# pytorch/ELF

Hardware: AMD Instinct MI355X
Metric: mcts_rollouts_per_sec (self-play, 19x19 Go, 8192 rollouts/move, bs 16) (higher is better)
Workload: dtype f32; 1 GPU; BASELINE configs[2]: MCTS self-play bs=16, 8192 rollouts/move, 20x256 fp16 net on PyTorch-ROCm, 2048 games/GPU in 1 group(s), window crosses a move boundary; games_per_gpu=2048, groups=1, board_size=19, mcts_threads=1, net_dtype=fp16, moves_in_window=2048, nodes_per_game=12288, node_bytes=6626, live_nodes=6241478, largest_tree=8184

## Files before the change

elf_amd/_lib.py:

```python
import ctypes as C
import os

HERE = os.path.dirname(os.path.abspath(__file__))
LIB_PATH = os.path.join(HERE, "lib", "libelf_amd.so")
ZOBRIST_BIN = os.path.join(HERE, "data", "zobrist21.bin")

_lib = None

KERNEL_SOURCES = ("go_board.cuh", "mcts.cuh", "train.cuh", "stl_emul.h", "engine_host.h", "elf_amd.hip", "mcts_capi.hip", "train_capi.hip",
                  "net_epilogue.hip", "Makefile")


def kernel_source_hash():
    import hashlib
    h = hashlib.sha256()
    for name in KERNEL_SOURCES:
        with open(os.path.join(HERE, "csrc", name), "rb") as f:
            h.update(name.encode() + b"\0" + f.read() + b"\0")
    return h.hexdigest()[:16]

_vp, _i, _i64, _f, _sz = C.c_void_p, C.c_int, C.c_int64, C.c_float, C.c_size_t
SIGNATURES = {
    "elfgo_create": (_i, [_i, _i, _i, _vp, C.POINTER(_vp)]),
    "elfgo_destroy": (_i, [_vp]),
    "elfgo_board_size": (_i, [_vp]),
    "elfgo_capacity": (_i, [_vp]),
    "elfgo_slot_bytes": (_sz, [_vp]),
    "elfgo_sync": (_i, [_vp, _vp]),
    "elfgo_reset": (_i, [_vp, _vp, _i, _vp]),
    "elfgo_copy": (_i, [_vp, _vp, _vp, _i, _vp]),
    "elfgo_forward": (_i, [_vp, _vp, _vp, _i, _vp, _vp]),
    "elfgo_legal_mask": (_i, [_vp, _vp, _i, _vp, _vp]),
    "elfgo_extract_agz": (_i, [_vp, _vp, _vp, _i, _vp, _i64, _vp]),
    "elfgo_extract_agz_fmt": (_i, [_vp, _vp, _vp, _i, _vp, _i64, _i, _vp]),
    "elfgo_evaluate": (_i, [_vp, _vp, _i, _f, _vp, _vp]),
    "elfgo_info": (_i, [_vp, _vp, _i, _vp, _vp]),
    "elfgo_export_board": (_i, [_vp, _vp, _i, _vp, _vp, _vp]),
    "elfgo_playout": (_i, [_vp, _vp, _vp, _i, _i, _vp, _vp]),
    "elfgo_setup": (_i, [_vp, _vp, _vp, _vp, _i, _vp, _vp]),
    "elfgo_area_map": (_i, [_vp, _vp, _i, _vp, _vp]),
    "elfgo_ladder_map": (_i, [_vp, _vp, _i, _vp, _vp, _vp]),
    "elfgo_own_create": (_i, [_vp, _i, C.POINTER(_vp)]),
    "elfgo_own_destroy": (_i, [_vp]),
    "elfgo_own_scratch_bytes": (_sz, [_vp]),
    "elfgo_own_run": (_i, [_vp, _vp, _vp, _i, _i, _i, _f, _vp, _vp, _vp]),
    "elfmcts_create": (_i, [_vp, _i, _i, _i, _vp, C.POINTER(_vp)]),
    "elfmcts_destroy": (_i, [_vp]),
    "elfmcts_set_options": (_i, [_vp, _vp]),
    "elfmcts_set_feature_format": (_i, [_vp, _i]),
    "elfmcts_get_feature_format": (_i, [_vp, C.POINTER(_i)]),
    "elfmcts_max_rollouts_per_step": (_i, []),
    "elfmcts_set_game_mask": (_i, [_vp, _vp]),
    "elfmcts_set_required_versions": (_i, [_vp, _vp]),
    "elfmcts_num_games": (_i, [_vp]),
    "elfmcts_edge_stride": (_i, [_vp]),
    "elfmcts_node_bytes": (_sz, [_vp]),
    "elfmcts_tree_bytes_per_game": (_sz, [_i, _i]),
    "elfmcts_tree_bytes_per_game2": (_sz, [_i, _i, _i, _i, _i]),
    "elfmcts_pool_info": (_i, [_vp, _vp, _i]),
    "elfmcts_count_live": (_i, [_vp, _vp]),
    "elfmcts_num_threads": (_i, [_vp]),
    "elfmcts_thread_draws": (_i, [_vp, _vp, _vp]),
    "elfmcts_clear": (_i, [_vp, _vp, _i, _vp]),
    "elfmcts_set_root": (_i, [_vp, _vp, _vp]),
    "elfmcts_set_d4": (_i, [_vp, _vp, _vp]),
    "elfmcts_dirichlet": (_i, [_vp, _vp, _vp, _f, _vp]),
    "elfmcts_select": (_i, [_vp, _vp, _vp, _i64, _vp, _vp]),
    "elfmcts_expand": (_i, [_vp, _vp, _i64, _vp, _vp, _i, _vp]),
    "elfmcts_root": (_i, [_vp, _vp, _vp, _vp, _vp, _vp, _vp, _vp]),
    "elfmcts_advance": (_i, [_vp, _vp, _vp]),
    "elfmcts_validate": (_i, [_vp, _vp]),
    "elfmcts_node_visits": (_i, [_vp, _vp]),
    "elfsp_create": (_i, [_vp, _i, _vp, C.POINTER(_vp)]),
    "elfsp_destroy": (_i, [_vp]),
    "elfsp_engine": (_vp, [_vp]),
    "elfsp_mcts": (_vp, [_vp]),
    "elfsp_ts_requests_deferred": (_i64, [_vp]),
    "elfsp_ts_games_deferred": (_i, [_vp]),
    "elfsp_max_rows": (_i, [_vp]),
    "elfsp_max_rows_actor": (_i, [_vp, _i]),
    "elfsp_mcts_actor": (_vp, [_vp, _i]),
    "elfsp_begin_step2": (_i, [_vp, _vp, _i64, _vp, _vp]),
    "elfsp_end_step2": (_i, [_vp, _vp, _i64, _vp, _vp, _vp]),
    "elfsp_last_rows2": (_i, [_vp, _vp]),
    "elfsp_set_request2": (_i, [_vp, _vp]),
    "elfsp_set_request3": (_i, [_vp, _vp, _vp]),
    "elfrec_sgf_parse": (_i, [_i, C.c_char_p, _vp, _vp, _i, _vp]),
    "elfrec_sgf_setup": (_i, [_i, C.c_char_p, _vp, _vp]),
    "elfrec_game_sgf": (_i64, [_vp, _vp, _i, _vp, _i, _f, C.c_char_p, C.c_char_p, C.c_char_p, C.c_char_p, _sz]),
    "elfrec_record_to_sgf": (_i64, [_vp, C.c_char_p, C.c_char_p, C.c_char_p, _sz, C.c_char_p, _sz]),
    "elfrec_client_create": (_i, [C.c_char_p, C.POINTER(_vp)]),
    "elfrec_client_destroy": (_i, [_vp]),
    "elfrec_client_feed": (_i, [_vp, C.c_char_p]),
    "elfrec_client_update_state": (_i, [_vp, _vp]),
    "elfrec_client_size": (_i, [_vp]),
    "elfrec_client_dump_and_clear": (_i64, [_vp, C.c_char_p, _sz]),
    "elfrec_parse_request_seq": (_i, [C.c_char_p, _vp, C.POINTER(_i64), _vp]),
    "elfrec_request_seq_to_json": (_i64, [_vp, _vp, _i64, C.c_char_p, _sz]),
    "elfsp_thread_states": (_i, [_vp, _vp, _i]),
    "elfrq_create": (_i, [_i, _i, _i, C.c_uint32, C.POINTER(_vp)]),
    "elfrq_destroy": (_i, [_vp]),
    "elfrq_insert": (_i, [_vp, C.c_int32, C.c_int32, _i, C.POINTER(C.c_int32)]),
    "elfrq_sizes": (_i, [_vp, _vp]),
    "elfrq_set_threads": (_i, [_vp, _i, _i64, C.c_uint64]),
    "elfrq_draw": (_i, [_vp, _i, _i, _vp, _vp, _vp]),
    "elfsp_progress": (_i, [_vp, _vp]),
    "elfsp_set_pick_seed": (_i, [_vp, C.c_uint32]),
    "elfsp_game_actor": (_i, [_vp, _i]),
    "elfsp_begin_step": (_i, [_vp, _vp, _i64, C.POINTER(_i), _vp]),
    "elfsp_end_step": (_i, [_vp, _vp, _i64, _vp, _vp, _vp]),
    "elfsp_last_rows": (_i, [_vp, C.POINTER(_i)]),
    "elfsp_set_request": (_i, [_vp, _i64, _i64, _f, _f, _i]),
    "elfsp_take_game_starts": (_i, [_vp, C.POINTER(_i64), C.POINTER(_i64)]),
    "elfsp_stats": (_i, [_vp, _vp]),
    "elfsp_games_finished": (_i64, [_vp]),
    "elfsp_search_log": (_i, [_vp, _i, _i, _vp, _vp, _vp, _vp, _vp]),
    "elfsp_play": (_i, [_vp, _vp, _vp]),
    "elfsp_preload": (_i, [_vp, _vp, _i, _i, _vp]),
    "elfsp_restart": (_i, [_vp, _vp, _i, _vp]),
    "elfsp_setup": (_i, [_vp, _vp, _i, _vp, _vp, _vp]),
    "elfsp_undo": (_i, [_vp, _vp, _i, _i, _vp]),
    "elfsp_finish": (_i, [_vp, _vp, _i, _i, _vp]),
    "elfsp_take_finished": (_i, [_vp, _vp, _i]),
    "elfsp_last_score": (_i, [_vp, _vp]),
    "elfsp_last_moves": (_i, [_vp, _vp]),
    "elfsp_records_pending": (_i, [_vp]),
    "elfsp_pop_record": (_i, [_vp, _vp, _sz, C.POINTER(_sz)]),
    "elftrain_create": (_i, [_vp, _i, _i, _i, C.c_uint32, C.POINTER(_vp)]),
    "elftrain_destroy": (_i, [_vp]),
    "elftrain_capacity": (_i, [_vp]),
    "elftrain_max_moves": (_i, [_vp]),
    "elftrain_num_records": (_i, [_vp]),
    "elftrain_put": (_i, [_vp, _i, _vp, _i, _f, _i64, _vp, _i, _vp, _i]),
    "elftrain_put_async": (_i, [_vp, _i, _vp, _i, _f, _i64, _vp, _i, _vp, _i, _vp]),
    "elftrain_set_keep_states": (_i, [_vp, _i]),
    "elftrain_draw": (_i, [_vp, _i, _i, _vp, _vp, _vp, _vp]),
    "elftrain_extract": (_i, [_vp, _vp, _vp, _vp, _i, _vp, _vp]),
    "elfrec_coords_to_sgfstr": (_i, [_i, _vp, _i, _vp, _sz]),
    "elfrec_sgfstr_to_coords": (_i, [_i, C.c_char_p, _vp, _i]),
    "elfrec_record_to_json": (_i, [_vp, _vp, _i, _vp, _i, _vp, _i, _f, _i, _i, C.c_uint64, C.c_uint64, _vp, _sz]),
    "elfrec_record_to_json2": (_i, [_vp, _vp, _vp, _i, _vp, _i, _vp, _i, _f, _i, _i, C.c_uint64, C.c_uint64, _vp, _sz]),
    "elfrec_quantise_policy": (_i, [_i, _vp, _vp, _i, _vp]),
    "elfnet_bias_act_f16": (_i, [_vp, _vp, _vp, _i64, _i, _i, _vp]),
    "elfnet_bias_act_bf16": (_i, [_vp, _vp, _vp, _i64, _i, _i, _vp]),
    "elfnet_conv3x3_f16": (_i, [_vp, _vp, _vp, _vp, _vp, _i64, _i, _i, _i, _i, _i, _i, _vp]),
    "elfnet_conv3x3_in_f16": (_i, [_vp, _vp, _vp, _vp, _i64, _i, _i, _i, _i, _i, _vp]),
    "elfnet_heads_workspace": (_sz, [_i64, _i, _i]),
    "elfnet_heads_f16": (_i, [_vp, _vp, _i64, _i, _i, _vp, _i64, _vp, _vp, _vp, _sz, _vp]),
    "elfgo_set_device": (_i, [_i]),
    "elfgo_get_device": (_i, [C.POINTER(_i)]),
    "elfgo_mem_info": (_i, [_i, C.POINTER(_sz), C.POINTER(_sz)]),
    "elfgo_pointer_kind": (_i, [_vp, C.POINTER(_i)]),
    "elfgo_memcpy2d_async": (_i, [_vp, _sz, _vp, _sz, _sz, _sz, _vp]),
    "elfgo_stream_sync": (_i, [_vp]),
    "elfgo_malloc": (_i, [C.POINTER(_vp), _sz]),
    "elfgo_free": (_i, [_vp]),
    "elfgo_memcpy_h2d": (_i, [_vp, _vp, _sz]),
    "elfgo_memcpy_d2h": (_i, [_vp, _vp, _sz]),
    "elfgo_error_string": (C.c_char_p, [_i]),
    "elfgo_version": (C.c_char_p, []),
}


class ElfNetHeads(C.Structure):
    _fields_ = [(n, _vp) for n in ("pconv_w", "pconv_b", "vconv_w", "vconv_b", "pi_w", "pi_b", "v1_w", "v1_b", "v2_w", "v2_b")] + \
               [("channels", C.c_int32), ("value_hidden", C.c_int32)]


def lib():
    global _lib
    if _lib is None:
        if not os.path.exists(LIB_PATH):
            raise ImportError(
                "elf_amd: %s not built. Run `python -c 'import __graft_entry__ as g; g.build()'` "
                "(or make -C elf_amd/csrc). There is no CPU fallback." % LIB_PATH
            )
        L = C.CDLL(LIB_PATH)
        for name, (res, args) in SIGNATURES.items():
            f = getattr(L, name)
            f.restype = res
            f.argtypes = args
        _lib = L
    return _lib


class ElfGoError(RuntimeError):
    pass


def check(status):
    if status != 0:
        raise ElfGoError("libelf_amd status %d: %s" % (status, lib().elfgo_error_string(status).decode()))
```

elf_amd/csrc/net_conv.hip:

```cpp
#include <hip/hip_runtime.h>
#include <stdint.h>

#include <array>

#if !__has_include("ck/ck.hpp")
#error "net_conv.hip needs Composable Kernel's headers (ck/ck.hpp, shipped with ROCm under <rocm>/include/ck): there is no build of libelf_amd.so without the fused trunk convolution"
#endif
#include "ck/ck.hpp"
#include "ck/tensor_operation/gpu/device/convolution_forward_specialization.hpp"
#include "ck/tensor_operation/gpu/device/gemm_specialization.hpp"
#include "ck/tensor_operation/gpu/device/impl/device_grouped_conv_fwd_multiple_abd_xdl_cshuffle.hpp"
#include "ck/tensor_operation/gpu/device/tensor_layout.hpp"
#include "ck/tensor_operation/gpu/element/element_wise_operation.hpp"

#include "../../include/elf_amd.h"

namespace {

using F16 = ck::half_t;
using F32 = float;
template <ck::index_t... Is>
using S = ck::Sequence<Is...>;
using PassThrough = ck::tensor_operation::element_wise::PassThrough;
namespace lay = ck::tensor_layout::convolution;

struct BiasResAct {
  int relu;
  template <typename E, typename C, typename D0>
  __host__ __device__ void operator()(E& e, const C& c, const D0& bias) const {
    float v = ck::type_convert<float>(ck::type_convert<F16>(c));
    v += ck::type_convert<float>(bias);
    if (relu) v = fmaxf(v, 0.0f);
    e = ck::type_convert<E>(v);
  }
  template <typename E, typename C, typename D0, typename D1>
  __host__ __device__ void operator()(E& e, const C& c, const D0& bias, const D1& res) const {
    float v = ck::type_convert<float>(ck::type_convert<F16>(c));
    v += ck::type_convert<float>(bias);
    v += ck::type_convert<float>(res);
    if (relu) v = fmaxf(v, 0.0f);
    e = ck::type_convert<E>(v);
  }
};

constexpr auto kConvDefault = ck::tensor_operation::device::ConvolutionForwardSpecialization::Default;
constexpr auto kMNKPadding = ck::tensor_operation::device::GemmSpecialization::MNKPadding;

template <typename DsLayout, typename DsTypes>
using ConvA = ck::tensor_operation::device::DeviceGroupedConvFwdMultipleABD_Xdl_CShuffle<
    2, lay::NHWGC, lay::GKYXC, DsLayout, lay::NHWGK, F16, F16, F32, F16, DsTypes, F16, PassThrough, PassThrough, BiasResAct,
    kConvDefault, kMNKPadding, 1, 256, 256, 128, 32, 8, 8, 32, 32, 4, 2,
    S<4, 64, 1>, S<1, 0, 2>, S<1, 0, 2>, 2, 8, 8, 1,
    S<4, 64, 1>, S<1, 0, 2>, S<1, 0, 2>, 2, 8, 8, 1,
    1, 1, S<1, 32, 1, 8>, 8>;

using DsBias = ck::Tuple<lay::G_K>;
using DsBiasRes = ck::Tuple<lay::G_K, lay::NHWGK>;
using T1 = ck::Tuple<F16>;
using T2 = ck::Tuple<F16, F16>;

struct DevGuard {
  int prev = -1;
  explicit DevGuard(int dev) {
    int cur = -1;
    if (hipGetDevice(&cur) == hipSuccess && cur != dev && hipSetDevice(dev) == hipSuccess) prev = cur;
  }
  ~DevGuard() { if (prev >= 0) (void)hipSetDevice(prev); }
  DevGuard(const DevGuard&) = delete;
  DevGuard& operator=(const DevGuard&) = delete;
};

struct Shape { int n, h, w, c, k; };

template <typename Op, int ND>
int run(const void* x, const void* w, const std::array<const void*, ND>& ds, void* y, const Shape& s, int relu, hipStream_t stream,
        bool launch) {
  using A5 = std::array<ck::index_t, 5>;
  using A2 = std::array<ck::index_t, 2>;
  const int n = s.n, h = s.h, wd = s.w, c = s.c, k = s.k;
  const A5 xl{1, n, c, h, wd}, xs{c, h * wd * c, 1, wd * c, c};
  const A5 wl{1, k, c, 3, 3}, ws{k * 9 * c, 9 * c, 1, 3 * c, c};
  const A5 yl{1, n, k, h, wd}, ys{k, h * wd * k, 1, wd * k, k};
  const A5 bs{k, 0, 1, 0, 0};
  std::array<A5, ND> dl, dst;
  dl[0] = yl; dst[0] = bs;
  if (ND == 2) { dl[ND - 1] = yl; dst[ND - 1] = ys; }
  const A2 one{1, 1};
  try {
    auto arg = Op::MakeArgument(x, w, ds, y, xl, xs, wl, ws, dl, dst, yl, ys, one, one, one, one, PassThrough{}, PassThrough{},
                                BiasResAct{relu});
    if (!Op::IsSupportedArgument(arg)) return ELFGO_E_BADARG;
    if (!launch) return 0;
    auto inv = Op::MakeInvoker();
    (void)inv.Run(arg, StreamConfig{stream, false});
  } catch (...) {
    hipError_t e = hipGetLastError();
    return e == hipSuccess ? (int)hipErrorLaunchFailure : (int)e;
  }
  hipError_t e = hipGetLastError();
  return e == hipSuccess ? 0 : (int)e;
}

}

extern "C" __attribute__((visibility("hidden"))) int elfnet_conv3x3_native_f16(const void* x, const void* w, const void* bias,
                                                                               const void* res, void* y, int64_t rows, int h, int wd,
                                                                               int c, int k, int relu, hipStream_t stream);

extern "C" int elfnet_conv3x3_f16(const void* x, const void* w, const void* bias, const void* res, void* y, int64_t rows, int h, int wd,
                                  int c, int k, int relu, int algo, void* stream) {
  if (!x || !w || !bias || !y || rows < 0 || h <= 0 || wd <= 0 || c <= 0 || k <= 0) return ELFGO_E_BADARG;
  if ((c & 7) != 0 || (k & 7) != 0 || (algo != 0 && algo != 1)) return ELFGO_E_BADARG;
  if ((((uintptr_t)x | (uintptr_t)w | (uintptr_t)bias | (uintptr_t)res | (uintptr_t)y) & 15) != 0) return ELFGO_E_BADARG;
  if (y == x || y == res) return ELFGO_E_BADARG;
  const int64_t cmax = c > k ? c : k;
  if (rows * h * wd * cmax >= ((int64_t)1 << 30) || (int64_t)k * 9 * c >= ((int64_t)1 << 30)) return ELFGO_E_BADARG;
  if (rows == 0) return 0;
  hipPointerAttribute_t at;
  if (hipPointerGetAttributes(&at, x) != hipSuccess) { (void)hipGetLastError(); return ELFGO_E_BADARG; }
  DevGuard _dg(at.device);
  const Shape s{(int)rows, h, wd, c, k};
  hipStream_t st = (hipStream_t)stream;
  if (algo == 1) return elfnet_conv3x3_native_f16(x, w, bias, res, y, rows, h, wd, c, k, relu, st);
  if (res) return run<ConvA<DsBiasRes, T2>, 2>(x, w, {bias, res}, y, s, relu, st, true);
  return run<ConvA<DsBias, T1>, 1>(x, w, {bias}, y, s, relu, st, true);
}
```

elf_amd/csrc/net_conv3x3.hip:

```cpp
#include <hip/hip_runtime.h>
#include <stdint.h>

#include "../../include/elf_amd.h"


namespace {

typedef _Float16 half8 __attribute__((ext_vector_type(8)));
typedef _Float16 half4 __attribute__((ext_vector_type(4)));
typedef float floatx16 __attribute__((ext_vector_type(16)));

constexpr int kTileM = 256;
constexpr int kTileN = 256;
constexpr int kThreads = 512;
constexpr int kOperandBytes = 256 * 128;
constexpr int kBufBytes = 2 * kOperandBytes;
constexpr int kLdsBytes = 2 * kBufBytes;

__device__ __attribute__((aligned(128))) unsigned char g_zero_line[128] = {0};

typedef const __attribute__((address_space(1))) void* gptr_t;
typedef __attribute__((address_space(3))) void* lptr_t;

__device__ __forceinline__ void stage16(const char* src, char* lds_base) {
  __builtin_amdgcn_global_load_lds((gptr_t)src, (lptr_t)lds_base, 16, 0, 0);
}

template <int kN, bool kLgkm>
__device__ __forceinline__ void wait_staged() {
  if constexpr (kLgkm) asm volatile("s_waitcnt vmcnt(%0) lgkmcnt(0)" ::"n"(kN) : "memory");
  else asm volatile("s_waitcnt vmcnt(%0)" ::"n"(kN) : "memory");
}
__device__ __forceinline__ void raw_barrier() {
  __builtin_amdgcn_s_barrier();
  asm volatile("" ::: "memory");
  __builtin_amdgcn_sched_barrier(0);
}
template <int kV> struct Mode { static constexpr int v = kV; };

template <bool kHasRes>
__global__ __launch_bounds__(kThreads, 2) void k_conv3x3_f16(const char* __restrict__ x, const char* __restrict__ w,
                                                             const _Float16* __restrict__ bias, const _Float16* __restrict__ res,
                                                             _Float16* __restrict__ y, int M, int H, int W, int Cin, int K, int relu) {
  __shared__ __attribute__((aligned(128))) char lds[kLdsBytes];
  const int tid = threadIdx.x, lane = tid & 63, wv = __builtin_amdgcn_readfirstlane(tid >> 6);
  const int kbase = blockIdx.y * kTileN;
  const int tile = blockIdx.x;

  uint32_t xoff[4], woff[4], xmask[4];
  const unsigned char* zsrc = g_zero_line + (lane & 7) * 16;
#pragma unroll
  for (int j = 0; j < 4; ++j) {
    const int hf = j >> 1, i = j & 1;
    const int r = i * 128 + hf * 64 + wv * 8 + (lane >> 3);
    const int p = tile * kTileM + r;
    uint32_t m = 0;
    if (p < M) {
      const int rem = p % (H * W), hh = rem / W, ww = rem - hh * W;
#pragma unroll
      for (int tap = 0; tap < 9; ++tap) {
        const int dy = tap / 3 - 1, dx = tap % 3 - 1;
        if ((unsigned)(hh + dy) < (unsigned)H && (unsigned)(ww + dx) < (unsigned)W) m |= 1u << tap;
      }
    }
    xmask[j] = m;
    xoff[j] = (uint32_t)p * (uint32_t)(Cin * 2) + (((lane & 7) ^ ((r >> 1) & 7)) << 4);
    const int rw = (i * 2 + (wv >> 2)) * 64 + hf * 32 + (wv & 3) * 8 + (lane >> 3);
    woff[j] = (uint32_t)(kbase + rw) * (uint32_t)(9 * Cin * 2) + (((lane & 7) ^ ((rw >> 1) & 7)) << 4);
  }
  auto stage_x = [&](int hf, int tap, int kc, int buf) {
    const int dy = tap / 3 - 1, dx = tap - (tap / 3) * 3 - 1;
    const uint32_t d = (uint32_t)((dy * W + dx) * Cin * 2 + kc * 128);
#pragma unroll
    for (int i = 0; i < 2; ++i)
      stage16(((xmask[hf * 2 + i] >> tap) & 1) ? x + (uint32_t)(xoff[hf * 2 + i] + d) : (const char*)zsrc,
              lds + buf * kBufBytes + (i * 128 + hf * 64 + wv * 8) * 128);
  };
  auto stage_w = [&](int hf, int tap, int kc, int buf) {
    const uint32_t d = (uint32_t)(tap * Cin * 2 + kc * 128);
#pragma unroll
    for (int i = 0; i < 2; ++i)
      stage16(w + (uint32_t)(woff[hf * 2 + i] + d),
              lds + buf * kBufBytes + kOperandBytes + ((i * 2 + (wv >> 2)) * 64 + hf * 32 + (wv & 3) * 8) * 128);
  };

  const int wm = wv >> 2, wn = wv & 3;
  const int fr = lane & 31, fh = lane >> 5;
  const int sw = (fr >> 1) & 7;
  const int xrow = (wm * 128 + fr) * 128;
  const int wrow = kOperandBytes + (wn * 64 + fr) * 128;
  int cs[4];
#pragma unroll
  for (int kk = 0; kk < 4; ++kk) cs[kk] = (((kk >> 1) * 4 + fh * 2 + (kk & 1)) ^ sw) << 4;
  auto ldx = [&](const char* b, int mt, int kk) { return *(const half8*)(b + xrow + mt * 4096 + cs[kk]); };
  auto ldw = [&](const char* b, int nt, int kk) { return *(const half8*)(b + wrow + nt * 4096 + cs[kk]); };

  floatx16 acc[4][2];
#pragma unroll
  for (int mt = 0; mt < 4; ++mt)
#pragma unroll
    for (int nt = 0; nt < 2; ++nt)
#pragma unroll
      for (int e = 0; e < 16; ++e) acc[mt][nt][e] = 0.0f;

  const int kchunks = Cin >> 6, ktiles = 9 * kchunks;
  half8 xf[2][4], wa[4], wb[4];
  int tap1 = 0, kc1 = 1, tap2 = 0, kc2 = 2;
  if (kchunks == 1) { tap1 = 1; kc1 = 0; tap2 = 2; kc2 = 0; }
  else if (kchunks == 2) { tap2 = 1; kc2 = 0; }
  stage_x(0, 0, 0, 0); stage_w(0, 0, 0, 0); stage_w(1, 0, 0, 0); stage_x(1, 0, 0, 0);
  stage_x(0, tap1, kc1, 1); stage_w(0, tap1, kc1, 1); stage_w(1, tap1, kc1, 1);
  wait_staged<8, false>();
  raw_barrier();

  auto ktile = [&](auto mode, int t) {
    constexpr int kMode = decltype(mode)::v;
    const int cur = t & 1, nxt = cur ^ 1;
    const char* b = lds + cur * kBufBytes;
#pragma unroll
    for (int kk = 0; kk < 4; ++kk) {
      wa[kk] = ldw(b, 0, kk);
      xf[0][kk] = ldx(b, 0, kk);
      xf[1][kk] = ldx(b, 1, kk);
      wb[kk] = ldw(b, 1, kk);
    }
    if constexpr (kMode <= 1) stage_x(1, tap1, kc1, nxt);
    wait_staged<kMode == 2 ? 0 : 8, true>();
    raw_barrier();
    __builtin_amdgcn_s_setprio(1);
#pragma unroll
    for (int kk = 0; kk < 4; ++kk) {
      acc[0][0] = __builtin_amdgcn_mfma_f32_32x32x16_f16(wa[kk], xf[0][kk], acc[0][0], 0, 0, 0);
      acc[1][0] = __builtin_amdgcn_mfma_f32_32x32x16_f16(wa[kk], xf[1][kk], acc[1][0], 0, 0, 0);
      acc[0][1] = __builtin_amdgcn_mfma_f32_32x32x16_f16(wb[kk], xf[0][kk], acc[0][1], 0, 0, 0);
      acc[1][1] = __builtin_amdgcn_mfma_f32_32x32x16_f16(wb[kk], xf[1][kk], acc[1][1], 0, 0, 0);
    }
    __builtin_amdgcn_s_setprio(0);
    __builtin_amdgcn_sched_barrier(0);
    raw_barrier();
#pragma unroll
    for (int kk = 0; kk < 4; ++kk) {
      xf[0][kk] = ldx(b, 2, kk);
      xf[1][kk] = ldx(b, 3, kk);
    }
    if constexpr (kMode == 0) { stage_x(0, tap2, kc2, cur); stage_w(0, tap2, kc2, cur); stage_w(1, tap2, kc2, cur); }
    wait_staged<kMode == 0 ? 8 : kMode == 1 ? 2 : 0, true>();
    raw_barrier();
    __builtin_amdgcn_s_setprio(1);
#pragma unroll
    for (int kk = 0; kk < 4; ++kk) {
      acc[2][0] = __builtin_amdgcn_mfma_f32_32x32x16_f16(wa[kk], xf[0][kk], acc[2][0], 0, 0, 0);
      acc[3][0] = __builtin_amdgcn_mfma_f32_32x32x16_f16(wa[kk], xf[1][kk], acc[3][0], 0, 0, 0);
      acc[2][1] = __builtin_amdgcn_mfma_f32_32x32x16_f16(wb[kk], xf[0][kk], acc[2][1], 0, 0, 0);
      acc[3][1] = __builtin_amdgcn_mfma_f32_32x32x16_f16(wb[kk], xf[1][kk], acc[3][1], 0, 0, 0);
    }
    __builtin_amdgcn_s_setprio(0);
    __builtin_amdgcn_sched_barrier(0);
    raw_barrier();
  };
  const int late = __builtin_amdgcn_readfirstlane(tid >> 8);
  if (late) raw_barrier();
  for (int t = 0; t < ktiles - 2; ++t) {
    ktile(Mode<0>{}, t);
    tap1 = tap2; kc1 = kc2;
    if (++kc2 == kchunks) { kc2 = 0; ++tap2; }
  }
  ktile(Mode<1>{}, ktiles - 2);
  ktile(Mode<2>{}, ktiles - 1);
  if (!late) raw_barrier();

  __syncthreads();
#pragma unroll
  for (int mt = 0; mt < 4; ++mt)
#pragma unroll
    for (int nt = 0; nt < 2; ++nt) {
      const int pos = wm * 128 + mt * 32 + fr;
#pragma unroll
      for (int g = 0; g < 4; ++g) {
        const int ch = wn * 64 + nt * 32 + g * 8 + fh * 4;
        half4 hv;
#pragma unroll
        for (int e = 0; e < 4; ++e) hv[e] = (_Float16)acc[mt][nt][g * 4 + e];
        *(half4*)(lds + pos * 512 + (((ch >> 3) ^ (pos & 31)) << 4) + ((ch >> 2) & 1) * 8) = hv;
      }
    }
  const int q = tid & 31;
  const half8 bv = *(const half8*)(bias + kbase + q * 8);
  if constexpr (kHasRes) {
    half8 rv[16];
#pragma unroll
    for (int it = 0; it < 16; ++it) {
      const int p = tile * kTileM + it * 16 + (tid >> 5);
      rv[it] = *(const half8*)(res + (size_t)(p < M ? p : M - 1) * K + kbase + q * 8);
    }
    __syncthreads();
#pragma unroll
    for (int it = 0; it < 16; ++it) {
      const int pos = it * 16 + (tid >> 5);
      const int p = tile * kTileM + pos;
      const half8 cv = *(const half8*)(lds + pos * 512 + ((q ^ (pos & 31)) << 4));
      half8 ov;
#pragma unroll
      for (int e = 0; e < 8; ++e) {
        float v = (float)cv[e];
        v += (float)bv[e];
        v += (float)rv[it][e];
        if (relu) v = fmaxf(v, 0.0f);
        ov[e] = (_Float16)v;
      }
      if (p < M) *(half8*)(y + (size_t)p * K + kbase + q * 8) = ov;
    }
  } else {
    __syncthreads();
#pragma unroll 4
    for (int it = 0; it < 16; ++it) {
      const int pos = it * 16 + (tid >> 5);
      const int p = tile * kTileM + pos;
      if (p < M) {
        const half8 cv = *(const half8*)(lds + pos * 512 + ((q ^ (pos & 31)) << 4));
        half8 ov;
#pragma unroll
        for (int e = 0; e < 8; ++e) {
          float v = (float)cv[e];
          v += (float)bv[e];
          if (relu) v = fmaxf(v, 0.0f);
          ov[e] = (_Float16)v;
        }
        *(half8*)(y + (size_t)p * K + kbase + q * 8) = ov;
      }
    }
  }
}

}

extern "C" __attribute__((visibility("hidden"))) int elfnet_conv3x3_native_f16(const void* x, const void* w, const void* bias,
                                                                               const void* res, void* y, int64_t rows, int h, int wd,
                                                                               int c, int k, int relu, hipStream_t stream) {
  if ((c & 63) != 0 || (k & 255) != 0) return ELFGO_E_BADARG;
  const int64_t m = rows * h * wd;
  const dim3 grid((unsigned)((m + kTileM - 1) / kTileM), (unsigned)(k / kTileN));
  if (res)
    hipLaunchKernelGGL(k_conv3x3_f16<true>, grid, dim3(kThreads), 0, stream, (const char*)x, (const char*)w, (const _Float16*)bias,
                       (const _Float16*)res, (_Float16*)y, (int)m, h, wd, c, k, relu);
  else
    hipLaunchKernelGGL(k_conv3x3_f16<false>, grid, dim3(kThreads), 0, stream, (const char*)x, (const char*)w, (const _Float16*)bias,
                       (const _Float16*)nullptr, (_Float16*)y, (int)m, h, wd, c, k, relu);
  hipError_t e = hipGetLastError();
  return e == hipSuccess ? 0 : (int)e;
}
```

include/elf_amd.h:

```cpp
#ifndef ELF_AMD_H_
#define ELF_AMD_H_
#include <stddef.h>
#include <stdint.h>

#ifdef __cplusplus
extern "C" {
#endif

typedef struct ElfGoEngine ElfGoEngine;

#define ELFGO_E_BADARG (-1)
#define ELFGO_E_BADSIZE (-2)
#define ELFGO_E_NOMEM (-3)
#define ELFGO_E_NODATA (-4)

#define ELFGO_INFO_WORDS 16

int elfgo_create(int board_size, int capacity, int device, const uint64_t* zobrist_host, ElfGoEngine** out);
int elfgo_destroy(ElfGoEngine* e);
int elfgo_board_size(const ElfGoEngine* e);
int elfgo_capacity(const ElfGoEngine* e);
size_t elfgo_slot_bytes(const ElfGoEngine* e);
int elfgo_sync(ElfGoEngine* e, void* stream);

// ... 115 lines not shown
  int32_t following_pass;
  int32_t reserved1;
} ElfSpOptions;
#define ELFSP_PICK_MOST_VISITED 0
#define ELFSP_PICK_STRONGEST_PRIOR 1
#define ELFSP_PICK_UNIFORM_RANDOM 2
#define ELFSP_ACTOR_BLACK 0
#define ELFSP_ACTOR_WHITE 1

typedef struct ElfSpSearch {
  int32_t game, move_played, best_action, total_visits, n_edges;
  float root_value, max_score, predicted_value;
} ElfSpSearch;

int elfsp_create(const ElfSpOptions* opt, int device, const uint64_t* zobrist_host, ElfSelfPlay** out);
int elfsp_destroy(ElfSelfPlay* sp);
ElfGoEngine* elfsp_engine(ElfSelfPlay* sp);
ElfMcts* elfsp_mcts(ElfSelfPlay* sp);
int64_t elfsp_ts_requests_deferred(const ElfSelfPlay* sp);
int elfsp_ts_games_deferred(const ElfSelfPlay* sp);
int elfsp_max_rows(const ElfSelfPlay* sp);
int elfsp_max_rows_actor(const ElfSelfPlay* sp, int actor);
ElfMcts* elfsp_mcts_actor(ElfSelfPlay* sp, int actor);
int elfsp_begin_step(ElfSelfPlay* sp, void* s_dst, int64_t stride_elems, int* n_rows, void* stream);
int elfsp_end_step(ElfSelfPlay* sp, const float* pi, int64_t pi_stride_floats, const float* value, const int64_t* rv, void* stream);
int elfsp_last_rows(ElfSelfPlay* sp, int* n_rows);
int elfsp_begin_step2(ElfSelfPlay* sp, void* const* s_dst, int64_t stride_elems, int* n_rows, void* stream);
int elfsp_end_step2(ElfSelfPlay* sp, const float* const* pi, int64_t pi_stride_floats, const float* const* value,
                    const int64_t* const* rv, void* stream);
int elfsp_last_rows2(ElfSelfPlay* sp, int* n_rows);
typedef struct ElfTsOptions {
  int32_t max_num_moves, num_threads, num_rollouts_per_thread, num_rollouts_per_batch;
  int32_t verbose, verbose_time, persistent_tree, pick_method ;
  int64_t seed;
  float root_epsilon, root_alpha;
  int32_t virtual_loss;
  int32_t use_prior, unexplored_q_zero, root_unexplored_q_zero;
  float c_puct;
  char log_prefix[60];
} ElfTsOptions;
typedef struct ElfSpRequest {
  int64_t black_ver, white_ver;
  float black_resign_thres, white_resign_thres, never_resign_prob;
  int32_t num_game_thread_used;
  int32_t player_swap;
  int32_t async;
  int32_t client_type;
} ElfSpRequest;
int elfsp_set_request2(ElfSelfPlay* sp, const ElfSpRequest* request);
int elfsp_set_request3(ElfSelfPlay* sp, const ElfSpRequest* request, const ElfTsOptions* mcts_opt);
int elfsp_set_request(ElfSelfPlay* sp, int64_t black_ver, int64_t white_ver, float resign_thres, float never_resign_prob, int async);
int elfsp_set_pick_seed(ElfSelfPlay* sp, uint32_t seed);
int elfsp_progress(const ElfSelfPlay* sp, int64_t* out6);
int elfsp_game_actor(const ElfSelfPlay* sp, int game);
int elfsp_take_game_starts(ElfSelfPlay* sp, int64_t* black_ver, int64_t* white_ver);
int elfsp_stats(ElfSelfPlay* sp, int64_t* out);
int elfsp_play(ElfSelfPlay* sp, const int32_t* moves_host, void* stream);
int elfsp_preload(ElfSelfPlay* sp, const uint16_t* moves_host, int n, int move_to, void* stream);
int elfsp_setup(ElfSelfPlay* sp, const int32_t* games_host, int n, const uint8_t* stones_host,
                const uint8_t* next_player_host, void* stream);
int elfsp_undo(ElfSelfPlay* sp, const int32_t* games_host, int n, int count, void* stream);
#define ELFSP_FR_RESIGN 0
#define ELFSP_FR_TWO_PASSES 1
#define ELFSP_FR_MAX_STEP 2
#define ELFSP_FR_CLEAR 3
#define ELFSP_FR_ILLEGAL 4
int elfsp_finish(ElfSelfPlay* sp, const int32_t* games_host, int n, int reason, void* stream);
int elfsp_restart(ElfSelfPlay* sp, const int32_t* games_host, int n, void* stream);
int elfsp_take_finished(ElfSelfPlay* sp, float* out_host, int cap);
int elfsp_last_score(const ElfSelfPlay* sp, float* out_host);
int elfsp_last_moves(const ElfSelfPlay* sp, int32_t* out_host);
int elfsp_records_pending(const ElfSelfPlay* sp);
int elfsp_pop_record(ElfSelfPlay* sp, char* buf, size_t cap, size_t* len);
int64_t elfsp_games_finished(const ElfSelfPlay* sp);
int elfsp_search_log(const ElfSelfPlay* sp, int first, int n, ElfSpSearch* rec, int32_t* coord, int32_t* visits, float* prior,
                     float* reward);

typedef struct ElfReplay ElfReplay;

typedef struct ElfTrainBatch {
  void* s;
  int64_t s_stride;
  int32_t s_format;
  int32_t num_future_actions;
  int64_t* offline_a;
  float* winner;
  float* mcts_scores;
  float* predicted_value;
  int32_t* move_idx;
  int32_t* num_move;
  int32_t* aug_code;
  int64_t* selfplay_ver;
} ElfTrainBatch;

int elftrain_create(ElfGoEngine* e, int capacity, int max_moves, int with_policies, uint32_t seed, ElfReplay** out);
int elftrain_destroy(ElfReplay* r);
int elftrain_capacity(const ElfReplay* r);
int elftrain_max_moves(const ElfReplay* r);
int elftrain_num_records(const ElfReplay* r);
int elftrain_put(ElfReplay* r, int slot, const uint16_t* moves_host, int num_moves, float reward, int64_t black_ver,
                 const uint8_t* policies_host, int num_policies, const float* values_host, int num_values);
int elftrain_put_async(ElfReplay* r, int slot, const uint16_t* moves_host, int num_moves, float reward, int64_t black_ver,
                       const uint8_t* policies_host, int num_policies, const float* values_host, int num_values, void* stream);
int elftrain_set_keep_states(ElfReplay* r, int on);
int elftrain_draw(ElfReplay* r, int n, int num_future_actions, int32_t* rec, int32_t* move_to, int32_t* d4, void* stream);
typedef struct ElfSgfHeader {
  int32_t size, handi, winner ;
  float komi, win_margin;
} ElfSgfHeader;
int elfrec_sgf_parse(int board_size, const char* text, int32_t* players, uint16_t* coords, int cap, ElfSgfHeader* header);
int elfrec_sgf_setup(int board_size, const char* text, uint8_t* stones, ElfSgfHeader* header);
int64_t elfrec_game_sgf(const ElfSpOptions* opt, const uint16_t* moves, int num_moves, const float* values, int num_values,
                        float final_value, const char* filename, const char* git_hash, const char* git_staged, char* out, size_t cap);
int64_t elfrec_record_to_sgf(const ElfSpOptions* opt, const char* record_json, const char* prefix, char* name_out, size_t name_cap,
                             char* out, size_t cap);
typedef struct ElfThreadState {
  int32_t thread_id, seq, move_idx, reserved;
  int64_t black, white;
} ElfThreadState;
typedef struct ElfClientRecords ElfClientRecords;
int elfrec_client_create(const char* identity, ElfClientRecords** out);
int elfrec_client_destroy(ElfClientRecords* c);
int elfrec_client_feed(ElfClientRecords* c, const char* record_json);
int elfrec_client_update_state(ElfClientRecords* c, const ElfThreadState* state);
int elfrec_client_size(const ElfClientRecords* c);
int64_t elfrec_client_dump_and_clear(ElfClientRecords* c, char* out, size_t cap);
int elfrec_parse_request_seq(const char* json_text, ElfSpRequest* request, int64_t* seq, ElfTsOptions* mcts_opt);
int64_t elfrec_request_seq_to_json(const ElfSpRequest* request, const ElfTsOptions* mcts_opt, int64_t seq, char* out, size_t cap);
int elfsp_thread_states(const ElfSelfPlay* sp, ElfThreadState* out, int capacity);
typedef struct ElfReaderQueues ElfReaderQueues;
int elfrq_create(int num_reader, int queue_min_size, int queue_max_size, uint32_t insert_seed, ElfReaderQueues** out);
int elfrq_destroy(ElfReaderQueues* q);
int elfrq_insert(ElfReaderQueues* q, int32_t slot, int32_t num_moves, int black_win, int32_t* evicted);
int elfrq_sizes(const ElfReaderQueues* q, int32_t* per_queue);
int elfrq_set_threads(ElfReaderQueues* q, int num_threads, int64_t seed, uint64_t job_hash);
int elfrq_draw(ElfReaderQueues* q, int num_acts, int num_future_actions, int32_t* slot, int32_t* move_to, int32_t* d4);
int elftrain_extract(ElfReplay* r, const int32_t* rec, const int32_t* move_to, const int32_t* d4, int n, const ElfTrainBatch* out,
                     void* stream);

int elfrec_coords_to_sgfstr(int board_size, const uint16_t* coords, int n, char* out, size_t cap);
int elfrec_sgfstr_to_coords(int board_size, const char* sgf, uint16_t* out, int cap);
int elfrec_record_to_json(const ElfSpOptions* opt, const uint16_t* moves, int num_moves, const uint8_t* policies, int num_policies,
                          const float* values, int num_values, float reward, int never_resign, int seq, uint64_t thread_id,
                          uint64_t timestamp, char* out, size_t cap);
int elfrec_record_to_json2(const ElfSpOptions* opt, const ElfSpRequest* request, const uint16_t* moves, int num_moves,
                           const uint8_t* policies, int num_policies, const float* values, int num_values, float reward, int never_resign,
                           int seq, uint64_t thread_id, uint64_t timestamp, char* out, size_t cap);
int elfrec_quantise_policy(int board_size, const int32_t* coord, const float* prob, int n, uint8_t* out);

int elfnet_bias_act_f16(void* x, const void* bias, const void* res, int64_t rows, int channels, int relu, void* stream);
int elfnet_bias_act_bf16(void* x, const void* bias, const void* res, int64_t rows, int channels, int relu, void* stream);
int elfnet_conv3x3_f16(const void* x, const void* w, const void* bias, const void* res, void* y,
                       int64_t rows, int h, int wd, int c, int k, int relu, int algo, void* stream);

int elfnet_conv3x3_in_f16(const void* x, const void* w, const void* bias, void* y,
                          int64_t rows, int h, int wd, int c, int k, int relu, void* stream);

typedef struct ElfNetHeads {
  const void *pconv_w, *pconv_b;
  const void *vconv_w, *vconv_b;
  const void *pi_w, *pi_b;
  const void *v1_w, *v1_b;
  const void *v2_w, *v2_b;
  int32_t channels, value_hidden;
} ElfNetHeads;
size_t elfnet_heads_workspace(int64_t rows, int h, int wd);
int elfnet_heads_f16(const void* act, const ElfNetHeads* hd, int64_t rows, int h, int wd,
                     float* pi, int64_t pi_stride, float* value, float* logits,
                     void* workspace, size_t workspace_bytes, void* stream);

int elfgo_set_device(int device);
int elfgo_get_device(int* device);
int elfgo_mem_info(int device, size_t* free_bytes, size_t* total_bytes);
int elfgo_pointer_kind(const void* p, int* device);
int elfgo_memcpy2d_async(void* dst, size_t dst_pitch, const void* src, size_t src_pitch, size_t width_bytes, size_t rows, void* stream);
int elfgo_stream_sync(void* stream);
int elfgo_malloc(void** dptr, size_t bytes);
int elfgo_free(void* dptr);
int elfgo_memcpy_h2d(void* dst, const void* src_host, size_t bytes);
int elfgo_memcpy_d2h(void* dst_host, const void* src, size_t bytes);
const char* elfgo_error_string(int status);
const char* elfgo_version(void);

#ifdef __cplusplus
}
#endif
#endif
```

Measured before the change: 61010 rollouts/s.

## Split tail-wave conv3x3 tiles into half-width work items to balance last round

The native conv3x3 kernel now maps a flat work-item index to (tile, column, half). When the final wave across the device's CUs would be at most half full, the remaining tiles are split into two half-N-width items computed by a kNT=1 variant of the tile routine. This targets the wave-quantization tail in the trunk convolution at bs16 MCTS shapes. In exchange it adds more templated kernel code, a plan query API and a device CU-count lookup, and half tiles reload the full activation operand.

New measurement: 62050 rollouts/s, median of 6. +1.7%, better.

```diff
diff --git a/elf_amd/_lib.py b/elf_amd/_lib.py
--- a/elf_amd/_lib.py
+++ b/elf_amd/_lib.py
@@ -144,6 +144,8 @@
     "elfnet_bias_act_f16": (_i, [_vp, _vp, _vp, _i64, _i, _i, _vp]),
     "elfnet_bias_act_bf16": (_i, [_vp, _vp, _vp, _i64, _i, _i, _vp]),
     "elfnet_conv3x3_f16": (_i, [_vp, _vp, _vp, _vp, _vp, _i64, _i, _i, _i, _i, _i, _i, _vp]),
+    "elfnet_conv3x3_f16_width": (_i, [_vp, _vp, _vp, _vp, _vp, _i64, _i, _i, _i, _i, _i, _i, _i, _vp]),
+    "elfnet_conv3x3_f16_plan": (_i64, [_i64, _i, _i, _i64, C.POINTER(_i), C.POINTER(_i), C.POINTER(_i)]),
     "elfnet_conv3x3_in_f16": (_i, [_vp, _vp, _vp, _vp, _i64, _i, _i, _i, _i, _i, _vp]),
     "elfnet_heads_workspace": (_sz, [_i64, _i, _i]),
     "elfnet_heads_f16": (_i, [_vp, _vp, _i64, _i, _i, _vp, _i64, _vp, _vp, _vp, _sz, _vp]),
diff --git a/elf_amd/csrc/net_conv.hip b/elf_amd/csrc/net_conv.hip
--- a/elf_amd/csrc/net_conv.hip
+++ b/elf_amd/csrc/net_conv.hip
@@ -105,12 +105,18 @@
 
 extern "C" __attribute__((visibility("hidden"))) int elfnet_conv3x3_native_f16(const void* x, const void* w, const void* bias,
                                                                                const void* res, void* y, int64_t rows, int h, int wd,
-                                                                               int c, int k, int relu, hipStream_t stream);
+                                                                               int c, int k, int relu, int round_width,
+                                                                               hipStream_t stream);
 
 extern "C" int elfnet_conv3x3_f16(const void* x, const void* w, const void* bias, const void* res, void* y, int64_t rows, int h, int wd,
                                   int c, int k, int relu, int algo, void* stream) {
+  return elfnet_conv3x3_f16_width(x, w, bias, res, y, rows, h, wd, c, k, relu, algo, 0, stream);
+}
+
+extern "C" int elfnet_conv3x3_f16_width(const void* x, const void* w, const void* bias, const void* res, void* y, int64_t rows, int h,
+                                        int wd, int c, int k, int relu, int algo, int round_width, void* stream) {
   if (!x || !w || !bias || !y || rows < 0 || h <= 0 || wd <= 0 || c <= 0 || k <= 0) return ELFGO_E_BADARG;
-  if ((c & 7) != 0 || (k & 7) != 0 || (algo != 0 && algo != 1)) return ELFGO_E_BADARG;
+  if ((c & 7) != 0 || (k & 7) != 0 || (algo != 0 && algo != 1) || round_width < 0) return ELFGO_E_BADARG;
   if ((((uintptr_t)x | (uintptr_t)w | (uintptr_t)bias | (uintptr_t)res | (uintptr_t)y) & 15) != 0) return ELFGO_E_BADARG;
   if (y == x || y == res) return ELFGO_E_BADARG;
   const int64_t cmax = c > k ? c : k;
@@ -121,7 +127,7 @@
   DevGuard _dg(at.device);
   const Shape s{(int)rows, h, wd, c, k};
   hipStream_t st = (hipStream_t)stream;
-  if (algo == 1) return elfnet_conv3x3_native_f16(x, w, bias, res, y, rows, h, wd, c, k, relu, st);
+  if (algo == 1) return elfnet_conv3x3_native_f16(x, w, bias, res, y, rows, h, wd, c, k, relu, round_width, st);
   if (res) return run<ConvA<DsBiasRes, T2>, 2>(x, w, {bias, res}, y, s, relu, st, true);
   return run<ConvA<DsBias, T1>, 1>(x, w, {bias}, y, s, relu, st, true);
 }
diff --git a/elf_amd/csrc/net_conv3x3.hip b/elf_amd/csrc/net_conv3x3.hip
--- a/elf_amd/csrc/net_conv3x3.hip
+++ b/elf_amd/csrc/net_conv3x3.hip
@@ -1,5 +1,7 @@
 #include <hip/hip_runtime.h>
 #include <stdint.h>
+
+#include <atomic>
 
 #include "../../include/elf_amd.h"
 
@@ -38,14 +40,28 @@
 }
 template <int kV> struct Mode { static constexpr int v = kV; };
 
-template <bool kHasRes>
-__global__ __launch_bounds__(kThreads, 2) void k_conv3x3_f16(const char* __restrict__ x, const char* __restrict__ w,
-                                                             const _Float16* __restrict__ bias, const _Float16* __restrict__ res,
-                                                             _Float16* __restrict__ y, int M, int H, int W, int Cin, int K, int relu) {
-  __shared__ __attribute__((aligned(128))) char lds[kLdsBytes];
+struct WorkItem { int tile, col, half; };
+__host__ __device__ inline WorkItem work_item(int id, int tiles, int nfull) {
+  int half = -1;
+  if (id >= nfull) {
+    const int e = id - nfull;
+    id = nfull + (e >> 1);
+    half = e & 1;
+  }
+  const int col = id / tiles;
+  return WorkItem{id - col * tiles, col, half};
+}
+__host__ __device__ inline int full_items(int64_t total, int64_t width) {
+  const int64_t r = total % width;
+  return (int)(total >= width && r > 0 && 2 * r <= width ? total - r : total);
+}
+
+template <bool kHasRes, int kNT>
+__device__ __forceinline__ void conv_tile(char* lds, const char* __restrict__ x, const char* __restrict__ w,
+                                          const _Float16* __restrict__ bias, const _Float16* __restrict__ res,
+                                          _Float16* __restrict__ y, int M, int H, int W, int Cin, int K, int relu, int tile,
+                                          int kbase) {
   const int tid = threadIdx.x, lane = tid & 63, wv = __builtin_amdgcn_readfirstlane(tid >> 6);
-  const int kbase = blockIdx.y * kTileN;
-  const int tile = blockIdx.x;
 
   uint32_t xoff[4], woff[4], xmask[4];
   const unsigned char* zsrc = g_zero_line + (lane & 7) * 16;
@@ -65,7 +81,7 @@
     }
     xmask[j] = m;
     xoff[j] = (uint32_t)p * (uint32_t)(Cin * 2) + (((lane & 7) ^ ((r >> 1) & 7)) << 4);
-    const int rw = (i * 2 + (wv >> 2)) * 64 + hf * 32 + (wv & 3) * 8 + (lane >> 3);
+    const int rw = kNT == 2 ? (i * 2 + (wv >> 2)) * 64 + hf * 32 + (wv & 3) * 8 + (lane >> 3) : i * 64 + wv * 8 + (lane >> 3);
     woff[j] = (uint32_t)(kbase + rw) * (uint32_t)(9 * Cin * 2) + (((lane & 7) ^ ((rw >> 1) & 7)) << 4);
   }
   auto stage_x = [&](int hf, int tap, int kc, int buf) {
@@ -81,36 +97,41 @@
 #pragma unroll
     for (int i = 0; i < 2; ++i)
       stage16(w + (uint32_t)(woff[hf * 2 + i] + d),
-              lds + buf * kBufBytes + kOperandBytes + ((i * 2 + (wv >> 2)) * 64 + hf * 32 + (wv & 3) * 8) * 128);
+              lds + buf * kBufBytes + kOperandBytes +
+                  (kNT == 2 ? (i * 2 + (wv >> 2)) * 64 + hf * 32 + (wv & 3) * 8 : i * 64 + wv * 8) * 128);
   };
 
   const int wm = wv >> 2, wn = wv & 3;
   const int fr = lane & 31, fh = lane >> 5;
   const int sw = (fr >> 1) & 7;
   const int xrow = (wm * 128 + fr) * 128;
-  const int wrow = kOperandBytes + (wn * 64 + fr) * 128;
+  const int wrow = kOperandBytes + (wn * 32 * kNT + fr) * 128;
   int cs[4];
 #pragma unroll
   for (int kk = 0; kk < 4; ++kk) cs[kk] = (((kk >> 1) * 4 + fh * 2 + (kk & 1)) ^ sw) << 4;
   auto ldx = [&](const char* b, int mt, int kk) { return *(const half8*)(b + xrow + mt * 4096 + cs[kk]); };
   auto ldw = [&](const char* b, int nt, int kk) { return *(const half8*)(b + wrow + nt * 4096 + cs[kk]); };
 
-  floatx16 acc[4][2];
+  floatx16 acc[4][kNT];
 #pragma unroll
   for (int mt = 0; mt < 4; ++mt)
 #pragma unroll
-    for (int nt = 0; nt < 2; ++nt)
+    for (int nt = 0; nt < kNT; ++nt)
 #pragma unroll
       for (int e = 0; e < 16; ++e) acc[mt][nt][e] = 0.0f;
 
+  constexpr int kFly = 2 * (2 + kNT);
   const int kchunks = Cin >> 6, ktiles = 9 * kchunks;
-  half8 xf[2][4], wa[4], wb[4];
+  half8 xf[2][4], wa[4], wb[kNT == 2 ? 4 : 1];
   int tap1 = 0, kc1 = 1, tap2 = 0, kc2 = 2;
   if (kchunks == 1) { tap1 = 1; kc1 = 0; tap2 = 2; kc2 = 0; }
   else if (kchunks == 2) { tap2 = 1; kc2 = 0; }
-  stage_x(0, 0, 0, 0); stage_w(0, 0, 0, 0); stage_w(1, 0, 0, 0); stage_x(1, 0, 0, 0);
-  stage_x(0, tap1, kc1, 1); stage_w(0, tap1, kc1, 1); stage_w(1, tap1, kc1, 1);
-  wait_staged<8, false>();
+  stage_x(0, 0, 0, 0); stage_w(0, 0, 0, 0);
+  if constexpr (kNT == 2) stage_w(1, 0, 0, 0);
+  stage_x(1, 0, 0, 0);
+  stage_x(0, tap1, kc1, 1); stage_w(0, tap1, kc1, 1);
+  if constexpr (kNT == 2) stage_w(1, tap1, kc1, 1);
+  wait_staged<kFly, false>();
   raw_barrier();
 
   auto ktile = [&](auto mode, int t) {
@@ -122,18 +143,20 @@
       wa[kk] = ldw(b, 0, kk);
       xf[0][kk] = ldx(b, 0, kk);
       xf[1][kk] = ldx(b, 1, kk);
-      wb[kk] = ldw(b, 1, kk);
+      if constexpr (kNT == 2) wb[kk] = ldw(b, 1, kk);
     }
     if constexpr (kMode <= 1) stage_x(1, tap1, kc1, nxt);
-    wait_staged<kMode == 2 ? 0 : 8, true>();
+    wait_staged<kMode == 2 ? 0 : kFly, true>();
     raw_barrier();
     __builtin_amdgcn_s_setprio(1);
 #pragma unroll
     for (int kk = 0; kk < 4; ++kk) {
       acc[0][0] = __builtin_amdgcn_mfma_f32_32x32x16_f16(wa[kk], xf[0][kk], acc[0][0], 0, 0, 0);
       acc[1][0] = __builtin_amdgcn_mfma_f32_32x32x16_f16(wa[kk], xf[1][kk], acc[1][0], 0, 0, 0);
-      acc[0][1] = __builtin_amdgcn_mfma_f32_32x32x16_f16(wb[kk], xf[0][kk], acc[0][1], 0, 0, 0);
-      acc[1][1] = __builtin_amdgcn_mfma_f32_32x32x16_f16(wb[kk], xf[1][kk], acc[1][1], 0, 0, 0);
+      if constexpr (kNT == 2) {
+        acc[0][1] = __builtin_amdgcn_mfma_f32_32x32x16_f16(wb[kk], xf[0][kk], acc[0][1], 0, 0, 0);
+        acc[1][1] = __builtin_amdgcn_mfma_f32_32x32x16_f16(wb[kk], xf[1][kk], acc[1][1], 0, 0, 0);
+      }
     }
     __builtin_amdgcn_s_setprio(0);
     __builtin_amdgcn_sched_barrier(0);
@@ -143,16 +166,21 @@
       xf[0][kk] = ldx(b, 2, kk);
       xf[1][kk] = ldx(b, 3, kk);
     }
-    if constexpr (kMode == 0) { stage_x(0, tap2, kc2, cur); stage_w(0, tap2, kc2, cur); stage_w(1, tap2, kc2, cur); }
-    wait_staged<kMode == 0 ? 8 : kMode == 1 ? 2 : 0, true>();
+    if constexpr (kMode == 0) {
+      stage_x(0, tap2, kc2, cur); stage_w(0, tap2, kc2, cur);
+      if constexpr (kNT == 2) stage_w(1, tap2, kc2, cur);
+    }
+    wait_staged<kMode == 0 ? kFly : kMode == 1 ? 2 : 0, true>();
     raw_barrier();
     __builtin_amdgcn_s_setprio(1);
 #pragma unroll
     for (int kk = 0; kk < 4; ++kk) {
       acc[2][0] = __builtin_amdgcn_mfma_f32_32x32x16_f16(wa[kk], xf[0][kk], acc[2][0], 0, 0, 0);
       acc[3][0] = __builtin_amdgcn_mfma_f32_32x32x16_f16(wa[kk], xf[1][kk], acc[3][0], 0, 0, 0);
-      acc[2][1] = __builtin_amdgcn_mfma_f32_32x32x16_f16(wb[kk], xf[0][kk], acc[2][1], 0, 0, 0);
-      acc[3][1] = __builtin_amdgcn_mfma_f32_32x32x16_f16(wb[kk], xf[1][kk], acc[3][1], 0, 0, 0);
+      if constexpr (kNT == 2) {
+        acc[2][1] = __builtin_amdgcn_mfma_f32_32x32x16_f16(wb[kk], xf[0][kk], acc[2][1], 0, 0, 0);
+        acc[3][1] = __builtin_amdgcn_mfma_f32_32x32x16_f16(wb[kk], xf[1][kk], acc[3][1], 0, 0, 0);
+      }
     }
     __builtin_amdgcn_s_setprio(0);
     __builtin_amdgcn_sched_barrier(0);
@@ -170,35 +198,37 @@
   if (!late) raw_barrier();
 
   __syncthreads();
+  constexpr int kRowB = kNT * 256, kCm = kNT * 16 - 1;
+  constexpr int kQs = kNT == 2 ? 5 : 4, kIts = kNT * 8;
 #pragma unroll
   for (int mt = 0; mt < 4; ++mt)
 #pragma unroll
-    for (int nt = 0; nt < 2; ++nt) {
+    for (int nt = 0; nt < kNT; ++nt) {
       const int pos = wm * 128 + mt * 32 + fr;
 #pragma unroll
       for (int g = 0; g < 4; ++g) {
-        const int ch = wn * 64 + nt * 32 + g * 8 + fh * 4;
+        const int ch = wn * 32 * kNT + nt * 32 + g * 8 + fh * 4;
         half4 hv;
 #pragma unroll
         for (int e = 0; e < 4; ++e) hv[e] = (_Float16)acc[mt][nt][g * 4 + e];
-        *(half4*)(lds + pos * 512 + (((ch >> 3) ^ (pos & 31)) << 4) + ((ch >> 2) & 1) * 8) = hv;
-      }
-    }
-  const int q = tid & 31;
+        *(half4*)(lds + pos * kRowB + (((ch >> 3) ^ (pos & kCm)) << 4) + ((ch >> 2) & 1) * 8) = hv;
+      }
+    }
+  const int q = tid & kCm;
   const half8 bv = *(const half8*)(bias + kbase + q * 8);
   if constexpr (kHasRes) {
-    half8 rv[16];
-#pragma unroll
-    for (int it = 0; it < 16; ++it) {
-      const int p = tile * kTileM + it * 16 + (tid >> 5);
+    half8 rv[kIts];
+#pragma unroll
+    for (int it = 0; it < kIts; ++it) {
+      const int p = tile * kTileM + (it << (9 - kQs)) + (tid >> kQs);
       rv[it] = *(const half8*)(res + (size_t)(p < M ? p : M - 1) * K + kbase + q * 8);
     }
     __syncthreads();
 #pragma unroll
-    for (int it = 0; it < 16; ++it) {
-      const int pos = it * 16 + (tid >> 5);
+    for (int it = 0; it < kIts; ++it) {
+      const int pos = (it << (9 - kQs)) + (tid >> kQs);
       const int p = tile * kTileM + pos;
-      const half8 cv = *(const half8*)(lds + pos * 512 + ((q ^ (pos & 31)) << 4));
+      const half8 cv = *(const half8*)(lds + pos * kRowB + ((q ^ (pos & kCm)) << 4));
       half8 ov;
 #pragma unroll
       for (int e = 0; e < 8; ++e) {
@@ -213,11 +243,11 @@
   } else {
     __syncthreads();
 #pragma unroll 4
-    for (int it = 0; it < 16; ++it) {
-      const int pos = it * 16 + (tid >> 5);
+    for (int it = 0; it < kIts; ++it) {
+      const int pos = (it << (9 - kQs)) + (tid >> kQs);
       const int p = tile * kTileM + pos;
       if (p < M) {
-        const half8 cv = *(const half8*)(lds + pos * 512 + ((q ^ (pos & 31)) << 4));
+        const half8 cv = *(const half8*)(lds + pos * kRowB + ((q ^ (pos & kCm)) << 4));
         half8 ov;
 #pragma unroll
         for (int e = 0; e < 8; ++e) {
@@ -232,20 +262,66 @@
   }
 }
 
+template <bool kHasRes>
+__global__ __launch_bounds__(kThreads, 2) void k_conv3x3_f16(const char* __restrict__ x, const char* __restrict__ w,
+                                                             const _Float16* __restrict__ bias, const _Float16* __restrict__ res,
+                                                             _Float16* __restrict__ y, int M, int H, int W, int Cin, int K, int relu,
+                                                             int tiles, int nfull) {
+  __shared__ __attribute__((aligned(128))) char lds[kLdsBytes];
+  const WorkItem wi = work_item((int)(blockIdx.y * gridDim.x + blockIdx.x), tiles, nfull);
+  if (__builtin_amdgcn_readfirstlane(wi.half) >= 0) {
+    conv_tile<kHasRes, 1>(lds, x, w, bias, res, y, M, H, W, Cin, K, relu, wi.tile, wi.col * kTileN + wi.half * (kTileN / 2));
+    return;
+  }
+  conv_tile<kHasRes, 2>(lds, x, w, bias, res, y, M, H, W, Cin, K, relu, wi.tile, wi.col * kTileN);
+}
+
+int round_width_of_device() {
+  static std::atomic<int> cus[64];
+  int dev = 0;
+  if (hipGetDevice(&dev) != hipSuccess || dev < 0 || dev >= 64) { (void)hipGetLastError(); return 0; }
+  int n = cus[dev].load(std::memory_order_relaxed);
+  if (n == 0) {
+    if (hipDeviceGetAttribute(&n, hipDeviceAttributeMultiprocessorCount, dev) != hipSuccess || n <= 0) { (void)hipGetLastError(); return 0; }
+    cus[dev].store(n, std::memory_order_relaxed);
+  }
+  return n;
+}
+
 }
 
 extern "C" __attribute__((visibility("hidden"))) int elfnet_conv3x3_native_f16(const void* x, const void* w, const void* bias,
                                                                                const void* res, void* y, int64_t rows, int h, int wd,
-                                                                               int c, int k, int relu, hipStream_t stream) {
-  if ((c & 63) != 0 || (k & 255) != 0) return ELFGO_E_BADARG;
+                                                                               int c, int k, int relu, int round_width,
+                                                                               hipStream_t stream) {
+  if ((c & 63) != 0 || (k & 255) != 0 || round_width < 0) return ELFGO_E_BADARG;
   const int64_t m = rows * h * wd;
-  const dim3 grid((unsigned)((m + kTileM - 1) / kTileM), (unsigned)(k / kTileN));
+  const int tiles = (int)((m + kTileM - 1) / kTileM), cols = k / kTileN;
+  const int64_t total = (int64_t)tiles * cols;
+  const int width = round_width > 0 ? round_width : round_width_of_device();
+  const int nfull = width > 0 ? full_items(total, width) : (int)total;
+  const dim3 grid = nfull < total ? dim3((unsigned)(2 * total - nfull)) : dim3((unsigned)tiles, (unsigned)cols);
   if (res)
     hipLaunchKernelGGL(k_conv3x3_f16<true>, grid, dim3(kThreads), 0, stream, (const char*)x, (const char*)w, (const _Float16*)bias,
-                       (const _Float16*)res, (_Float16*)y, (int)m, h, wd, c, k, relu);
+                       (const _Float16*)res, (_Float16*)y, (int)m, h, wd, c, k, relu, tiles, nfull);
   else
     hipLaunchKernelGGL(k_conv3x3_f16<false>, grid, dim3(kThreads), 0, stream, (const char*)x, (const char*)w, (const _Float16*)bias,
-                       (const _Float16*)nullptr, (_Float16*)y, (int)m, h, wd, c, k, relu);
+                       (const _Float16*)nullptr, (_Float16*)y, (int)m, h, wd, c, k, relu, tiles, nfull);
   hipError_t e = hipGetLastError();
   return e == hipSuccess ? 0 : (int)e;
 }
+
+extern "C" int64_t elfnet_conv3x3_f16_plan(int64_t tiles, int columns, int round_width, int64_t id, int* tile, int* column, int* half) {
+  if (tiles <= 0 || columns <= 0 || round_width <= 0 || tiles * columns >= ((int64_t)1 << 30)) return ELFGO_E_BADARG;
+  const int64_t total = tiles * columns;
+  const int nfull = full_items(total, round_width);
+  const int64_t groups = 2 * total - nfull;
+  if (tile || column || half) {
+    if (id < 0 || id >= groups) return ELFGO_E_BADARG;
+    const WorkItem wi = work_item((int)id, (int)tiles, nfull);
+    if (tile) *tile = wi.tile;
+    if (column) *column = wi.col;
+    if (half) *half = wi.half;
+  }
+  return groups;
+}
diff --git a/include/elf_amd.h b/include/elf_amd.h
--- a/include/elf_amd.h
+++ b/include/elf_amd.h
@@ -291,6 +291,9 @@
 int elfnet_bias_act_bf16(void* x, const void* bias, const void* res, int64_t rows, int channels, int relu, void* stream);
 int elfnet_conv3x3_f16(const void* x, const void* w, const void* bias, const void* res, void* y,
                        int64_t rows, int h, int wd, int c, int k, int relu, int algo, void* stream);
+int elfnet_conv3x3_f16_width(const void* x, const void* w, const void* bias, const void* res, void* y,
+                             int64_t rows, int h, int wd, int c, int k, int relu, int algo, int round_width, void* stream);
+int64_t elfnet_conv3x3_f16_plan(int64_t tiles, int columns, int round_width, int64_t id, int* tile, int* column, int* half);
 
 int elfnet_conv3x3_in_f16(const void* x, const void* w, const void* bias, void* y,
                           int64_t rows, int h, int wd, int c, int k, int relu, void* stream);
```
